# automerge/automerge-classic

Measured on AMD Instinct MI355X. Metric: CRDT ops/sec applied (bulk replay), higher is better.
Workload: dtype u32

## Files before the change

### automerge_classic_amd/csrc/am355_api.hip

```cpp
#include "am355_ctx.h"
#include "am355_scan.h"
#include "am355_textrec.h"

static bool ctx_init(am355_ctx* c) {
  {
    unsigned hw = std::thread::hardware_concurrency();
    const char* env = getenv("AM355_HOST_THREADS");
    unsigned want = env && atoi(env) > 0 ? (unsigned)atoi(env) : std::min(hw ? hw : 4u, 64u);
    c->pool.reset(new HostPool(want > 1 ? want - 1 : 0));
  }
  int prio_low = 0, prio_high = 0;
  (void)hipDeviceGetStreamPriorityRange(&prio_low, &prio_high);
  auto make_stream = [](Stream& s, int prio) { return hipStreamCreateWithPriority(&s.h, hipStreamNonBlocking, prio) == hipSuccess; };
  if (!make_stream(c->stream, prio_high)) return false;
  {
    const char* env = getenv("AM355_HASH_CUS");
    int want = env ? atoi(env) : 0;
    bool made = false;
    if (want > 0) {
      hipDeviceProp_t prop;
      if (hipGetDeviceProperties(&prop, c->device) == hipSuccess && prop.multiProcessorCount > want) {
        int n_cu = prop.multiProcessorCount;
        std::vector<uint32_t> mask((size_t)(n_cu + 31) / 32, 0u);
        for (int k = 0; k < want; k++) { int cu = n_cu - 1 - k; mask[(size_t)cu / 32] |= 1u << (cu % 32); }
        made = hipExtStreamCreateWithCUMask(&c->stream2.h, (uint32_t)mask.size(), mask.data()) == hipSuccess;
      }
    }
    if (!made && !make_stream(c->stream2, prio_low)) return false;
  }
  if (!make_stream(c->stream3, prio_high) || !make_stream(c->stream4, prio_high)) return false;
  for (Event* e : {&c->ev_fork, &c->ev_join, &c->ev[0], &c->ev[1], &c->ev[2], &c->ev[3], &c->ev[4], &c->ev[5], &c->ev[6], &c->ev[7], &c->ev_parse, &c->ev_b0, &c->ev_b1,
                   &c->ev_counts, &c->ev_runs, &c->ev_s1, &c->ev_plan, &c->ev_tables, &c->ev_fills, &c->ev_sched})
    if (hipEventCreate(&e->h) != hipSuccess) return false;
  if (!c->h_sig.ensure(sizeof(HostSignals))) return false;
  memset(c->h_sig.p, 0, sizeof(HostSignals));
  if (const char* e = getenv("AM355_PHASE_EVENTS")) c->phase_events = strcmp(e, "0") != 0;
  return true;
}

extern "C" am355_ctx* am355_create(int device) {
  int n = 0;
  if (hipGetDeviceCount(&n) != hipSuccess || n <= 0 || device < 0 || device >= n) return nullptr;
  (void)hipSetDeviceFlags(hipDeviceScheduleSpin);
  if (hipSetDevice(device) != hipSuccess) return nullptr;
  am355_ctx* c = new am355_ctx();
  c->device = device;
  if (!ctx_init(c)) { delete c; return nullptr; }
  return c;
}

am355_ctx::~am355_ctx() {
  (void)hipSetDevice(device);
  if (lane) lane->wait();
  (void)doc_sum.wait();
  for (const Stream* s : {&stream, &stream2, &stream3, &stream4})
    if (s->h) (void)hipStreamSynchronize(s->h);
  if (shard_comm) (void)am355_shard_finalize(this);
}

extern "C" void am355_destroy(am355_ctx* c) {
  delete c;
}

extern "C" const char* am355_last_error(const am355_ctx* c) { return c ? c->err.c_str() : "no context (no GPU?)"; }
extern "C" uint32_t am355_flags(const am355_ctx* c) { return c ? c->flags : 0; }

extern "C" int am355_set_phase_events(am355_ctx* c, int on) {
  if (!c) return AM355_E_ARG;
  c->phase_events = on != 0;
  return AM355_OK;
}

extern "C" int am355_get_stats(const am355_ctx* c, am355_stats* out) {
  if (!c || !out) return AM355_E_ARG;
  *out = c->stats;
  return AM355_OK;
}

extern "C" int am355_get_hashes(const am355_ctx* c, uint8_t* out) {
  if (!c || !out) return AM355_E_ARG;
  if (!c->replayed || !c->h_hashes.p || c->is_document) return AM355_E_STATE;
  memcpy(out, c->h_hashes.p, 32 * (size_t)c->n_changes);
  return AM355_OK;
}

extern "C" int am355_arena_epoch(const am355_ctx* c, uint64_t* epoch) {
  if (!c || !epoch) return AM355_E_ARG;
  *epoch = c->arena_epoch;
  return AM355_OK;
}

extern "C" int am355_get_hashes_range(const am355_ctx* c, uint32_t first, uint32_t count, uint8_t* out) {
  if (!c || (!out && count)) return AM355_E_ARG;
  if (!c->replayed || !c->h_hashes.p || c->is_document) return AM355_E_STATE;
  if (first > c->n_changes || count > c->n_changes - first) return AM355_E_ARG;
  if (count) memcpy(out, (const uint8_t*)c->h_hashes.p + 32 * (size_t)first, 32 * (size_t)count);
  return AM355_OK;
}

extern "C" int am355_applied_in_input_order(const am355_ctx* c, int* yes) {
  if (!c || !yes) return AM355_E_ARG;
  if (!c->replayed || c->is_document) return AM355_E_STATE;
  bool ok = c->pending_change.empty() && c->n_pending == 0 && c->applied_change.size() == c->n_changes;
  for (uint32_t i = 0; ok && i < c->n_changes; i++) ok = c->applied_change[i] == i;
  *yes = ok ? 1 : 0;
  return AM355_OK;
}

extern "C" int am355_resident_counters(const am355_ctx* c, uint64_t out[3]) {
  if (!c || !out) return AM355_E_ARG;
  out[0] = c->n_resident_calls;
  out[1] = c->n_resident_fallbacks;
  out[2] = c->n_resorder_calls;
  return AM355_OK;
}
// ... 477 lines not shown
```

### automerge_classic_amd/csrc/am355_ctx.h

```cpp
#pragma once
#include "../../include/am355.h"
#include "am355_decode.h"
#include "am355_merge.h"
#include "am355_bigcol.h"
#include "am355_encode.h"
#include "am355_prims.h"
#include "am355_render.h"
#include "am355_host.h"
#include "am355_pinflate.h"
#include "am355_history.h"
#include "am355_delta.h"
#include "am355_resorder.h"
#include "am355_apply.h"
#include "am355_sync.h"
#include "am355_sched.h"
#include "am355_hist.h"
#include "am355_canary.h"

#include <zlib.h>

#include <algorithm>
#include <atomic>
#include <chrono>
#include <cstdarg>
// ... 255 lines not shown
  TraceLap(const char* prefix_, int width_, std::chrono::steady_clock::time_point t0_ = std::chrono::steady_clock::now())
      : on(getenv("AM355_TRACE") != nullptr), prefix(prefix_), width(width_), t0(t0_) {}
  void operator()(const char* what) const {
    if (on) fprintf(stderr, "%s %-*s +%8.3f ms\n", prefix, width, what, std::chrono::duration<double, std::milli>(std::chrono::steady_clock::now() - t0).count());
  }
};

struct SignalBlock {
  static constexpr uint32_t WORDS = 8;
  HostBuf h;
  uint32_t seq = 0;
  bool ready() { return h.ensure((WORDS + 1) * 4); }
  const uint32_t* words() { return h.as<uint32_t>(); }
  hipError_t fetch(const uint32_t* dev, uint32_t n, uint32_t k, hipStream_t st) {
    uint32_t* hw = h.as<uint32_t>();
    volatile uint32_t* hseq = hw + WORDS;
    if (seq == 0) *hseq = 0;
    launch_signal_words(dev, n, nullptr, 0, hw + k, hseq, ++seq, st);
    return wait_host_signal(hseq, seq, st) ? hipSuccess : hipMemcpy(hw + k, dev, 4 * (size_t)n, hipMemcpyDeviceToHost);
  }
};

struct LaneJoin {
  AsyncLane* l = nullptr;
  ~LaneJoin() { if (l) l->wait(); }
};

struct Hash32 {
  uint8_t b[32];
  bool operator==(const Hash32& o) const { return memcmp(b, o.b, 32) == 0; }
};
struct Hash32Hasher {
  size_t operator()(const Hash32& h) const { size_t v; memcpy(&v, h.b, sizeof v); return v; }
};

}
using namespace am355_host;

struct am355_ctx {
  ~am355_ctx();
  int device = 0;
  Stream stream;
  Stream stream2;
  Stream stream3;
  Stream stream4;
  Event ev_fork, ev_join;
  Event ev[8];
  Event ev_parse, ev_b0, ev_b1;
  Event ev_counts, ev_runs;
  std::string err;
  uint32_t flags = 0;

  PinnedBytes raw;
  std::unique_ptr<HostPool> pool;
  std::unique_ptr<AsyncLane> lane;
  std::vector<uint64_t> raw_off;
  uint32_t n_changes = 0;
  DevBuf d_plan_totals;
  bool spec_launched = false;
  bool spec_large_launched = false;
  uint32_t spec_cap_ops = 0, spec_cap_preds = 0;
  uint32_t hint_ops = 0, hint_preds = 0, hint_large = 0;
  bool staged = false, replayed = false, ir_fetched = false;
  int ir_copy_enqueued = 0;
  bool prefetch_ir = false;
  bool has_unknown_cols = false;
  bool staging_in_flight = false;
  bool is_document = false;
  ChangeMeta doc_meta{};
  std::vector<uint32_t> doc_actor_rank;
  DevBuf d_arena, d_offsets, d_metas;
  uint64_t arena_epoch = 1;
  CopyRanges pending_up;
  std::vector<uint32_t> breaks_dev;
  void* breaks_dev_ptr = nullptr;
  HostBuf h_breaks_ahead;
  bool offsets_on_device = false;
  HostBuf h_metas, h_offsets, h_sig;
  uint32_t sig_seq = 0;
  Event ev_s1;
  Event ev_fills;
  Event ev_sched;
  Event ev_plan, ev_tables;
  void* counts_zeroed_at = nullptr; size_t counts_zeroed = 0;
  bool phase_events = false;
  DevBuf d_big, d_bigvals, d_ks;
  HostBuf h_biginfo;
  BigColDesc doc_cols{};
  bool doc_serial = false;
  DevBuf d_entries, d_amap_base, d_amap_prov, d_slots, d_first_idx, d_hashes, d_hash_tab, d_min_idx, d_has_dep, d_words, d_slot_rank, d_scan1, d_plan_sums, d_dep_idx, d_self_idx, d_rank_ids;
  HostBuf h_dep_idx, h_self_idx, h_amap, h_amap_base;
  HostBuf h_slots, h_hashes, h_has_dep, h_words, h_stage, h_s1;
  DevBuf d_s1;
  ChangeBrief* hp_briefs = nullptr;
  uint32_t* hp_distinct = nullptr;
  bool have_host_metas = false;
  uint32_t amap_cap = 0, slot_mask = 0, hash_mask = 0;
  bool used_fast_path = false;

  std::vector<ChangePlan> plans;
  std::vector<uint32_t> applied_change, applied_op_base;
  struct DocSum {
    static constexpr size_t PIECE = (size_t)4 << 20;
    std::thread t;
    std::unique_ptr<std::atomic<uint8_t>[]> copied;
    size_t n_pieces = 0;
    bool pending = false, ok = false;
    bool wait() {
      if (t.joinable()) t.join();
      pending = false;
      return ok;
    }
    ~DocSum() { if (t.joinable()) t.join(); }
  } doc_sum;
  std::vector<uint8_t> doc_bytes;
  std::vector<uint8_t> saved;
  HistoryOutput history;
  bool history_ok = false; uint32_t history_flags = 0;
  std::vector<std::vector<uint8_t>> inflate_scratch;
  std::vector<std::unique_ptr<PInflateJob>> pinflate_jobs;
  std::vector<uint32_t> doc_col_rows;
  std::vector<std::pair<uint32_t, std::vector<uint8_t>>> doc_chg_cols;
  std::vector<uint8_t> doc_tail;
  bool doc_other_ops_cols = false;
  DevBuf d_save, d_enc, d_encout;
  HostBuf h_encout;
  std::vector<uint32_t> amap;
  std::vector<ActorSpan> spans;
  std::vector<uint32_t> actor_tab_off;
  std::vector<std::string> actors;
  std::vector<uint32_t> clock_actor;
  std::vector<uint64_t> clock_seq;
  std::vector<uint8_t> heads;
  uint32_t n_applied = 0, n_pending = 0;
  uint64_t n_ops = 0, n_preds = 0, max_op = 0;
  DevBuf d_plans, d_amap, d_tables;
  ActorSpan* p_spans = nullptr;
  uint32_t* p_tab_off = nullptr;

  DevBuf d_cols, d_pred, d_merge, d_sort, d_ir, d_counts;
  OpCols cols{};
  MergeBufs mb{};
  PatchIR ir{};
  HostBuf h_counts;
  Counts counts{};

  HostBuf h_ir, h_rows;
  am355_patch_ir hir{};
  std::vector<uint32_t> actor_off;
  std::vector<uint8_t> actor_bytes;
  std::string json;

  am355_stats stats{};

  std::vector<uint32_t> pending_change;
  std::vector<uint32_t> pass_first_row;
  DevBuf d_delta, d_pass, d_delta_edit, d_sched, d_hist;
  HostBuf h_sched;
  bool key_unbounded = false;
  bool device_scheduled = false;
  HostBuf h_delta;
  DeltaBufs delta{};
  bool h_tables_current = false, h_tables_were_current = false;
  bool batch_list_only = false;
  void* apply_tail = nullptr;
  ApplyPatch apply;
// ... 207 lines not shown
```

### automerge_classic_amd/csrc/am355_stage.hip

```cpp
#include "am355_ctx.h"
#include "am355_pinflate.h"

bool read_uleb_host(const uint8_t* p, size_t len, size_t& off, uint64_t& out) {
  uint64_t v = 0;
  int shift = 0;
  while (off < len && shift < 64) {
    uint8_t b = p[off++];
    v |= (uint64_t)(b & 0x7f) << shift;
    shift += 7;
    if (!(b & 0x80)) { out = v; return true; }
  }
  return false;
}

constexpr size_t INFLATE_CAP = 0xfff00000ull;

int flush_uploads(am355_ctx* c) {
  if (!c->pending_up.n) return AM355_OK;
  launch_copy_ranges(c->pending_up, c->stream);
  c->pending_up.n = 0;
  HIPCHK(c, hipGetLastError());
  return AM355_OK;
}

int queue_upload(am355_ctx* c, void* dst, const void* src, size_t bytes) {
  if (!bytes) return AM355_OK;
  static const bool off = getenv("AM355_NO_UPLOAD_QUEUE") != nullptr;
  if (off || bytes > ((size_t)256 << 10)) {
    int rc = flush_uploads(c);
    if (rc) return rc;
    HIPCHK(c, hipMemcpyAsync(dst, src, bytes, hipMemcpyHostToDevice, c->stream));
    return AM355_OK;
  }
  if (c->pending_up.n == LAUNCH_RANGES) { int rc = flush_uploads(c); if (rc) return rc; }
  if (!c->pending_up.add(dst, src, bytes)) return fail(c, AM355_E_DEVICE, "upload queue full");
  return AM355_OK;
}

int upload_offsets(am355_ctx* c) {
  if (c->offsets_on_device) return AM355_OK;
  const size_t bytes = sizeof(uint64_t) * ((size_t)c->n_changes + 1);
  if (!c->d_offsets.ensure(bytes) || !c->h_offsets.ensure(bytes)) return fail(c, AM355_E_NOMEM, "device allocation failed");
  memcpy(c->h_offsets.p, c->raw_off.data(), bytes);
  HIPCHK(c, hipMemcpyAsync(c->d_offsets.p, c->h_offsets.p, bytes, hipMemcpyHostToDevice, c->stream));
  c->offsets_on_device = true;
  return AM355_OK;
}

int load_changes_impl(am355_ctx* c, const uint8_t* arena, const uint64_t* offsets, uint32_t n, bool keep_staged) {
  if (!c || (!arena && n) || !offsets) return c ? fail(c, AM355_E_ARG, "null argument") : AM355_E_ARG;
  (void)hipSetDevice(c->device);
  (void)c->doc_sum.wait();
  const uint32_t k0 = keep_staged ? c->n_changes : 0;
  const size_t b0 = keep_staged ? c->raw.size() : 0;
  { int frc = flush_uploads(c); if (frc) return frc; }
  if (c->staging_in_flight) { c->staging_in_flight = false; HIPCHK(c, hipStreamSynchronize(c->stream)); }
  c->staged = c->replayed = c->ir_fetched = false;
  if (!keep_staged) { c->resident_valid = false; c->arena_epoch++; }
  c->apply_ready = false;
  c->state_checked = false;
  c->is_document = false;
  c->flags = 0;
  if (n && offsets[n] - offsets[0] >= ((uint64_t)1 << 20))
    c->pool->prewake(offsets[1] - offsets[0] > 9 && arena[offsets[0] + 8] == 2 ? c->pool->size() : 4);
  for (uint32_t i = 0; i < n; i++)
    if (offsets[i] > offsets[i + 1]) return fail(c, AM355_E_ARG, "change offsets must be ascending (offsets[%u] > offsets[%u])", i, i + 1);
  if (offsets[n] - offsets[0] + b0 >= INFLATE_CAP) { c->flags |= AM355_F_OVERFLOW; return fail(c, AM355_E_UNSUPPORTED, "batch larger than 4 GiB (32-bit arena offsets)"); }
  const size_t in_bytes = (size_t)(offsets[n] - offsets[0]);
  const bool trace = getenv("AM355_TRACE") != nullptr;
  auto t_begin = std::chrono::steady_clock::now();
  auto lap = [&](const char* what) {
    if (trace) fprintf(stderr, "load_changes: %-22s +%8.3f ms\n", what, std::chrono::duration<double, std::milli>(std::chrono::steady_clock::now() - t_begin).count());
  };
  unsigned n_slices = 1;
  const char* slice_env = getenv("AM355_SLICE_BYTES");
  const size_t slice_bytes = slice_env && atol(slice_env) > 0 ? (size_t)atol(slice_env) : (size_t)1 << 21;
  const bool deflated = n && ((offsets[1] - offsets[0] > 9 && arena[offsets[0] + 8] == 2) || (offsets[n / 2 + 1] - offsets[n / 2] > 9 && arena[offsets[n / 2] + 8] == 2));
  const size_t per_slice = deflated && !slice_env ? (size_t)64 << 10 : slice_bytes;
  if (in_bytes >= 2 * per_slice && n >= 16)
    n_slices = (unsigned)std::min<size_t>({(size_t)(c->pool->size() + 1) * (deflated ? 8 : 2), in_bytes / per_slice, (size_t)n / 8});
  if (n_slices < 1) n_slices = 1;
  struct Slice { uint32_t c0 = 0, c1 = 0; size_t out_bytes = 0, base = 0; bool any_deflated = false; int err = 0; uint32_t err_change = 0; std::vector<uint8_t> tmp; std::vector<uint32_t> tmp_len; };
  std::vector<Slice> slices(n_slices);
  {
    uint32_t ci = 0;
    for (unsigned k = 0; k < n_slices; k++) {
      slices[k].c0 = ci;
      uint64_t target = offsets[0] + (uint64_t)in_bytes * (k + 1) / n_slices;
      while (ci < n && (k + 1 == n_slices || offsets[ci + 1] <= target)) ci++;
      slices[k].c1 = ci;
    }
    slices[n_slices - 1].c1 = n;
  }
  auto phase_a = [&](unsigned k) {
    Slice& sl = slices[k];
    for (uint32_t i = sl.c0; i < sl.c1; i++) {
      size_t len = (size_t)(offsets[i + 1] - offsets[i]);
      if (len > 9 && arena[offsets[i] + 8] == 2) { sl.any_deflated = true; break; }
    }
    if (!sl.any_deflated) { sl.out_bytes = (size_t)(offsets[sl.c1] - offsets[sl.c0]); return; }
    sl.tmp_len.resize(sl.c1 - sl.c0);
    std::vector<uint8_t> out;
    for (uint32_t i = sl.c0; i < sl.c1 && !sl.err; i++) {
      const uint8_t* p = arena + offsets[i];
      size_t len = (size_t)(offsets[i + 1] - offsets[i]);
      size_t before = sl.tmp.size();
      if (len > 9 && p[8] == 2) {
        size_t off = 9;
        uint64_t clen;
        if (!read_uleb_host(p, len, off, clen) || clen > len - off) { sl.err = 10; sl.err_change = i; break; }
        int irc = inflate_raw(p + off, (size_t)clen, out, INFLATE_CAP);
        if (irc) { sl.err = irc; sl.err_change = i; break; }
        sl.tmp.insert(sl.tmp.end(), p, p + 8);
        sl.tmp.push_back(1);
        uint64_t v = out.size();
        do { uint8_t x = v & 0x7f; v >>= 7; if (v) x |= 0x80; sl.tmp.push_back(x); } while (v);
        sl.tmp.insert(sl.tmp.end(), out.begin(), out.end());
      } else {
        sl.tmp.insert(sl.tmp.end(), p, p + len);
      }
      if (sl.tmp.size() >= INFLATE_CAP) { sl.err = 2; sl.err_change = i; break; }
      sl.tmp_len[i - sl.c0] = (uint32_t)(sl.tmp.size() - before);
    }
    sl.out_bytes = sl.tmp.size();
  };
  c->pool->run(n_slices, phase_a);
  lap("inflate / sizes");
  size_t total = 0;
  for (Slice& sl : slices) {
    if (sl.err == 10) { c->flags |= AM355_F_BAD_CHUNK; return fail(c, AM355_E_INVALID, "change %u: bad deflate container", sl.err_change); }
    if (sl.err == 3) return fail(c, AM355_E_NOMEM, "inflate: out of memory");
    if (sl.err == 2) { c->flags |= AM355_F_OVERFLOW; return fail(c, AM355_E_UNSUPPORTED, "change %u: inflated size beyond the 4 GiB batch limit", sl.err_change); }
    if (sl.err) { c->flags |= AM355_F_BAD_DEFLATE; return fail(c, AM355_E_INVALID, "change %u: invalid or truncated deflate data", sl.err_change); }
    sl.base = total;
    total += sl.out_bytes;
    if (total + b0 >= INFLATE_CAP) { c->flags |= AM355_F_OVERFLOW; return fail(c, AM355_E_UNSUPPORTED, "batch larger than 4 GiB (32-bit arena offsets)"); }
  }
  const uint32_t n_all = k0 + n;
  c->raw.resize(b0 + total);
  c->raw_off.resize((size_t)n_all + 1);
  c->raw_off[n_all] = b0 + total;
  c->n_changes = n_all;
  if (!(keep_staged ? c->d_arena.ensure_keep(b0 + total + 64, b0) : c->d_arena.ensure(total + 64)) || !c->d_offsets.ensure(sizeof(uint64_t) * ((size_t)n_all + 1)) ||
      !(keep_staged ? c->d_metas.ensure_keep(sizeof(ChangeMeta) * (size_t)std::max(n_all, 1u), sizeof(ChangeMeta) * (size_t)k0)
                    : c->d_metas.ensure(sizeof(ChangeMeta) * (size_t)std::max(n_all, 1u))) || !c->h_metas.ensure(sizeof(ChangeMeta) * (size_t)std::max(n_all, 1u)) ||
      !c->d_counts.ensure(sizeof(Counts)) || !c->h_counts.ensure(2 * sizeof(Counts)) || !c->h_offsets.ensure(sizeof(uint64_t) * ((size_t)n_all + 1)))
    return fail(c, AM355_E_NOMEM, "device allocation failed");
  uint8_t* raw = c->raw.data() + b0;
  uint8_t* d_raw = c->d_arena.as<uint8_t>() + b0;
  uint64_t* roff = c->raw_off.data() + k0;
  std::vector<hipError_t> h2d(n_slices, hipSuccess);
  bool any_deflated = false;
  for (const Slice& sl : slices) any_deflated = any_deflated || sl.any_deflated;
  const char* gather_env = getenv("AM355_GATHER_UNIT");
  if (!any_deflated && (total >= ((size_t)4 << 20) || (gather_env && total > 0))) {
    const size_t unit = gather_env && atol(gather_env) > 0 ? (size_t)atol(gather_env) : (size_t)256 << 10;
    const size_t n_units = (total + unit - 1) / unit;
    std::vector<uint32_t> group_of(n_units);
    std::vector<size_t> group_first;
    for (size_t u = 0, span = 1; u < n_units; span = std::min<size_t>(span * 2, 64)) {
      group_first.push_back(u);
      for (size_t k = 0; k < span && u < n_units; k++, u++) group_of[u] = (uint32_t)group_first.size() - 1;
    }
    const size_t n_groups = group_first.size();
    group_first.push_back(n_units);
    std::vector<std::atomic<uint32_t>> left(n_groups);
    for (size_t g = 0; g < n_groups; g++) left[g].store((uint32_t)(group_first[g + 1] - group_first[g]));
    h2d.assign(n_groups, hipSuccess);
    const uint8_t* src = arena + offsets[0];
    const uint64_t off0 = offsets[0];
    std::atomic<size_t> next_unit{0};
    const unsigned n_helpers = (unsigned)std::min<size_t>(4, std::min<size_t>(n_units > 1 ? n_units - 1 : 0, c->pool->size()));
    lap("  buffers ready");
    c->pool->run(n_helpers + 1, [&](unsigned task) {
      const bool issuer = task == 0;
      size_t next_group = 0;
      auto issue_ready = [&]() {
        while (next_group < n_groups && left[next_group].load(std::memory_order_acquire) == 0) {
          size_t gb = group_first[next_group] * unit, ge = std::min(total, group_first[next_group + 1] * unit);
          h2d[next_group] = hipMemcpyAsync(d_raw + gb, raw + gb, ge - gb, hipMemcpyHostToDevice, c->stream);
          if (trace) fprintf(stderr, "load_changes:   group %zu (%zu KiB) enqueued +%8.3f ms\n", next_group, (ge - gb) >> 10, std::chrono::duration<double, std::milli>(std::chrono::steady_clock::now() - t_begin).count());
          next_group++;
        }
      };
      if (issuer) (void)hipSetDevice(c->device);
      for (;;) {
        size_t u = next_unit.fetch_add(1, std::memory_order_relaxed);
        if (u >= n_units) break;
        size_t b = u * unit, e = std::min(total, b + unit);
        memcpy(raw + b, src + b, e - b);
        left[group_of[u]].fetch_sub(1, std::memory_order_acq_rel);
        if (issuer) issue_ready();
      }
      if (issuer) {
        while (next_group < n_groups) {
          issue_ready();
#if defined(__x86_64__)
          __builtin_ia32_pause();
#endif
        }
      }
    });
    for (uint32_t i = 0; i < n; i++) roff[i] = b0 + (offsets[i] - off0);
  } else {
    std::vector<uint32_t> group_of(n_slices);
    std::vector<size_t> group_begin{0};
    {
      size_t acc = 0;
      for (unsigned k = 0; k < n_slices; k++) {
        group_of[k] = (uint32_t)group_begin.size() - 1;
        acc += slices[k].out_bytes;
        if (acc >= ((size_t)2 << 20) && k + 1 < n_slices) { group_begin.push_back(slices[k + 1].base); acc = 0; }
      }
      group_begin.push_back(total);
    }
    const size_t n_groups = group_begin.size() - 1;
    std::vector<std::atomic<uint32_t>> left(n_groups);
    for (auto& x : left) x.store(0);
    for (unsigned k = 0; k < n_slices; k++) left[group_of[k]].fetch_add(1);
    h2d.assign(n_groups, hipSuccess);
    if (n_slices == 1) {
      Slice& sl = slices[0];
      if (sl.any_deflated) {
        if (sl.out_bytes) memcpy(raw, sl.tmp.data(), sl.out_bytes);
        size_t o = b0;
        for (uint32_t i = 0; i < n; i++) { roff[i] = o; o += sl.tmp_len[i]; }
      } else {
        if (sl.out_bytes) memcpy(raw, arena + offsets[0], sl.out_bytes);
        for (uint32_t i = 0; i < n; i++) roff[i] = b0 + (offsets[i] - offsets[0]);
      }
      if (total) {
        if (keep_staged) { int qrc = queue_upload(c, d_raw, raw, total); if (qrc) return qrc; }
        else h2d[0] = hipMemcpyAsync(d_raw, raw, total, hipMemcpyHostToDevice, c->stream);
      }
    } else
    c->pool->run(n_slices + 1, [&](unsigned task) {
      if (task == 0) {
        (void)hipSetDevice(c->device);
        for (size_t g = 0; g < n_groups; g++) {
          while (left[g].load(std::memory_order_acquire) != 0) {
#if defined(__x86_64__)
            __builtin_ia32_pause();
#endif
          }
          size_t gb = group_begin[g], ge = group_begin[g + 1];
          if (ge > gb) h2d[g] = hipMemcpyAsync(d_raw + gb, raw + gb, ge - gb, hipMemcpyHostToDevice, c->stream);
        }
        return;
      }
      Slice& sl = slices[task - 1];
      if (sl.any_deflated) {
        if (sl.out_bytes) memcpy(raw + sl.base, sl.tmp.data(), sl.out_bytes);
        size_t o = b0 + sl.base;
        for (uint32_t i = sl.c0; i < sl.c1; i++) { roff[i] = o; o += sl.tmp_len[i - sl.c0]; }
      } else {
        if (sl.out_bytes) memcpy(raw + sl.base, arena + offsets[sl.c0], sl.out_bytes);
        for (uint32_t i = sl.c0; i < sl.c1; i++) roff[i] = b0 + sl.base + (offsets[i] - offsets[sl.c0]);
      }
      left[group_of[task - 1]].fetch_sub(1, std::memory_order_acq_rel);
    });
  }
  lap("gathered, H2D enqueued");
  for (hipError_t e : h2d)
    if (e != hipSuccess) return fail(c, AM355_E_DEVICE, "hipMemcpyAsync (arena): %s", hipGetErrorString(e));
  c->offsets_on_device = false;
  if (!keep_staged) { int orc = upload_offsets(c); if (orc) return orc; }
  c->staging_in_flight = true;
  static const bool stage_sync = getenv("AM355_STAGE_SYNC") != nullptr;
  if (trace || stage_sync) { c->staging_in_flight = false; HIPCHK(c, hipStreamSynchronize(c->stream)); lap("H2D done"); }
  c->staged = true;
  c->stats = am355_stats{};
  c->stats.n_changes = n_all;
  c->stats.raw_bytes = c->raw.size();
  return AM355_OK;
}

namespace {
struct HostRle {
  const uint8_t* p; size_t len, off = 0; int64_t count = 0; int state = 0; int64_t last = 0; bool last_null = true; bool is_signed;
  HostRle(const uint8_t* p_, size_t l, bool sg) : p(p_), len(l), is_signed(sg) {}
  bool done() const { return count == 0 && off >= len; }
  bool leb(bool sg, int64_t& out) {
    uint64_t v = 0; int shift = 0;
    while (off < len && shift < 64) {
      uint8_t b = p[off++];
// ... 391 lines not shown
```

### automerge_classic_amd/engine.py

```python
import ctypes
import os

import numpy as np

_HERE = os.path.dirname(os.path.abspath(__file__))
DEFAULT_LIB = os.path.join(_HERE, "csrc", "libam355.so")

AM355_OK = 0
AM355_E_DEVICE, AM355_E_ARG, AM355_E_INVALID, AM355_E_UNSUPPORTED, AM355_E_STATE, AM355_E_NOMEM = -1, -2, -3, -4, -5, -6

FLAG_NAMES = {
    1 << 0: "BAD_MAGIC", 1 << 1: "BAD_CHECKSUM", 1 << 2: "BAD_CHUNK", 1 << 3: "BAD_COLUMNS", 1 << 4: "BAD_LEB", 1 << 5: "BAD_RLE",
    1 << 6: "BAD_ROW", 1 << 7: "UNKNOWN_OBJECT", 1 << 8: "BAD_ELEM", 1 << 9: "BAD_PRED", 1 << 10: "DUP_OPID", 1 << 11: "BAD_COUNTER",
    1 << 12: "UNSUPPORTED", 1 << 13: "OVERFLOW", 1 << 16: "BAD_SEQ", 1 << 17: "UNKNOWN_ACTOR", 1 << 18: "BAD_DEFLATE",
}


class Stats(ctypes.Structure):
    _fields_ = [
        ("n_changes", ctypes.c_uint32), ("n_applied", ctypes.c_uint32), ("n_pending", ctypes.c_uint32),
        ("n_actors", ctypes.c_uint32), ("n_objects", ctypes.c_uint32), ("n_heads", ctypes.c_uint32),
        ("n_ops", ctypes.c_uint64), ("max_op", ctypes.c_uint64), ("raw_bytes", ctypes.c_uint64),
        ("n_map_values", ctypes.c_uint64), ("n_list_elems", ctypes.c_uint64), ("n_edits", ctypes.c_uint64),
        ("ir_bytes", ctypes.c_uint64),
# ... 327 lines not shown
        L.am355_resident_new_actor_calls.restype = ctypes.c_int
    if hasattr(L, "am355_set_resident_new_objects"):
        L.am355_set_resident_new_objects.argtypes = [vp, ctypes.c_int]
        L.am355_set_resident_new_objects.restype = ctypes.c_int
        L.am355_resident_new_object_calls.argtypes = [vp, vp]
        L.am355_resident_new_object_calls.restype = ctypes.c_int
    if hasattr(L, "am355_set_resident_counters"):
        L.am355_set_resident_counters.argtypes = [vp, ctypes.c_int]
        L.am355_set_resident_counters.restype = ctypes.c_int
        L.am355_resident_counter_calls.argtypes = [vp, vp]
        L.am355_resident_counter_calls.restype = ctypes.c_int
    if hasattr(L, "am355_set_resident_map_merge"):
        L.am355_set_resident_map_merge.argtypes = [vp, ctypes.c_int]
        L.am355_set_resident_map_merge.restype = ctypes.c_int
        L.am355_resident_map_merge_calls.argtypes = [vp, vp]
        L.am355_resident_map_merge_calls.restype = ctypes.c_int
    if hasattr(L, "am355_apply_local_change"):
        L.am355_encode_change.argtypes = [vp, ctypes.POINTER(LocalChange), ctypes.POINTER(ctypes.c_void_p), ctypes.POINTER(ctypes.c_size_t), vp]
        L.am355_apply_local_change.argtypes = [vp, ctypes.POINTER(LocalChange), ctypes.POINTER(ctypes.c_void_p), ctypes.POINTER(ctypes.c_size_t)]
        L.am355_local_change_calls.argtypes = [vp, vp]
        for f in ("am355_encode_change", "am355_apply_local_change", "am355_local_change_calls"):
            getattr(L, f).restype = ctypes.c_int
    if hasattr(L, "am355_set_local_small"):
        L.am355_set_local_small.argtypes = [vp, ctypes.c_int]
        L.am355_set_local_small.restype = ctypes.c_int
        L.am355_local_small_calls.argtypes = [vp, vp]
        L.am355_local_small_calls.restype = ctypes.c_int
    if hasattr(L, "am355_changes_added"):
        L.am355_find_changes.argtypes = [vp, vp, u32, vp]
        for f in ("am355_changes_since", "am355_changes_added", "am355_missing_deps"):
            getattr(L, f).argtypes = [vp, vp, u32, ctypes.POINTER(ctypes.c_void_p), ctypes.POINTER(u32)]
        L.am355_set_graph_probe_min.argtypes = [vp, u32]
        L.am355_graph_query_calls.argtypes = [vp, vp]
        L.am355_test_hash_probe.argtypes = [vp, vp, u32, vp, u32, vp]
        for f in ("am355_find_changes", "am355_changes_since", "am355_changes_added", "am355_missing_deps", "am355_set_graph_probe_min", "am355_graph_query_calls",
                  "am355_test_hash_probe"):
            getattr(L, f).restype = ctypes.c_int
    if hasattr(L, "am355_object_text"):
        L.am355_object_text.argtypes = [vp, ctypes.c_uint64, vp, ctypes.c_size_t, ctypes.POINTER(ctypes.c_void_p), ctypes.POINTER(ctypes.c_size_t), ctypes.POINTER(TextInfo)]
        L.am355_object_text_calls.argtypes = [vp, vp]
        L.am355_set_text_pinned_max.argtypes = [vp, ctypes.c_uint64]
        L.am355_text_limits.argtypes = [vp]
        for f in ("am355_object_text", "am355_object_text_calls", "am355_set_text_pinned_max", "am355_text_limits"):
            getattr(L, f).restype = ctypes.c_int
    if hasattr(L, "am355_text_splice"):
        L.am355_text_locate.argtypes = [vp, ctypes.c_uint64, vp, ctypes.c_size_t, ctypes.c_uint64, ctypes.c_uint64, ctypes.POINTER(ctypes.c_void_p), ctypes.POINTER(u32),
                                        ctypes.POINTER(ctypes.c_uint64)]
        L.am355_text_splice.argtypes = [vp, ctypes.c_uint64, vp, ctypes.c_size_t, ctypes.c_uint64, ctypes.c_uint64, vp, vp, u32, vp, ctypes.c_size_t, ctypes.c_int64, vp, u32,
                                        ctypes.POINTER(ctypes.c_void_p), ctypes.POINTER(ctypes.c_size_t)]
        L.am355_text_splice_calls.argtypes = [vp, vp]
        L.am355_text_locate_limits.argtypes = [vp]
        for f in ("am355_text_locate", "am355_text_splice", "am355_text_splice_calls", "am355_text_locate_limits"):
            getattr(L, f).restype = ctypes.c_int
    if hasattr(L, "am355_list_splice"):
        pvp, psz = ctypes.POINTER(ctypes.c_void_p), ctypes.POINTER(ctypes.c_size_t)
        L.am355_list_locate.argtypes = [vp, ctypes.c_uint64, vp, ctypes.c_size_t, ctypes.c_uint64, ctypes.c_uint64, pvp, ctypes.POINTER(u32), pvp, ctypes.POINTER(u32),
                                        ctypes.POINTER(ctypes.c_uint64)]
        L.am355_list_splice.argtypes = [vp, ctypes.c_uint64, vp, ctypes.c_size_t, ctypes.c_uint64, ctypes.c_uint64, vp, u32, vp, u32, vp, ctypes.c_size_t, ctypes.c_int64, vp, u32,
                                        pvp, psz]
        L.am355_list_set.argtypes = [vp, ctypes.c_uint64, vp, ctypes.c_size_t, ctypes.c_uint64, vp, vp, u32, vp, ctypes.c_size_t, ctypes.c_int64, vp, u32, pvp, psz]
        L.am355_list_splice_calls.argtypes = [vp, vp]
        L.am355_list_locate_limits.argtypes = [vp]
        L.am355_test_list_premises.argtypes = [vp, vp, u32, u32, u32, u32, ctypes.POINTER(u32), ctypes.POINTER(u32)]
        for f in ("am355_list_locate", "am355_list_splice", "am355_list_set", "am355_list_splice_calls", "am355_list_locate_limits", "am355_test_list_premises"):
            getattr(L, f).restype = ctypes.c_int
    if hasattr(L, "am355_text_position"):
        L.am355_text_position.argtypes = [vp, ctypes.c_uint64, vp, ctypes.c_size_t, vp, u32, ctypes.POINTER(ctypes.c_void_p), ctypes.POINTER(ctypes.c_uint64)]
        L.am355_rank_of_actor.argtypes = [vp, vp, ctypes.c_size_t, ctypes.POINTER(u32)]
        L.am355_actor_of_rank.argtypes = [vp, u32, ctypes.POINTER(ctypes.c_void_p), ctypes.POINTER(ctypes.c_size_t)]
        L.am355_actor_of_rank.restype = ctypes.c_int
        L.am355_text_position_calls.argtypes = [vp, vp]
        L.am355_text_position_limits.argtypes = [vp]
        for f in ("am355_text_position", "am355_rank_of_actor", "am355_text_position_calls", "am355_text_position_limits"):
            getattr(L, f).restype = ctypes.c_int
    if hasattr(L, "am355_map_update"):
        pvp, psz = ctypes.POINTER(ctypes.c_void_p), ctypes.POINTER(ctypes.c_size_t)
        L.am355_map_locate.argtypes = [vp, ctypes.c_uint64, vp, ctypes.c_size_t, vp, vp, u32, pvp, pvp, ctypes.POINTER(u32)]
        L.am355_map_update.argtypes = [vp, ctypes.c_uint64, vp, ctypes.c_size_t, vp, u32, vp, u32, vp, u32, vp, ctypes.c_size_t, ctypes.c_int64, vp, u32, pvp, psz]
        L.am355_map_calls.argtypes = [vp, vp]
        L.am355_map_locate_limits.argtypes = [vp]
        L.am355_set_map_locate_thread.argtypes = [vp, ctypes.c_int]
        for f in ("am355_map_locate", "am355_map_update", "am355_map_calls", "am355_map_locate_limits", "am355_set_map_locate_thread"):
            getattr(L, f).restype = ctypes.c_int
    L.am355_get_raw.argtypes = [vp, ctypes.POINTER(ctypes.c_void_p), ctypes.POINTER(ctypes.c_void_p), ctypes.POINTER(u32)]
    L.am355_doc_changes.argtypes = [vp, u32, ctypes.POINTER(ctypes.c_void_p), ctypes.POINTER(ctypes.c_void_p), ctypes.POINTER(u32), ctypes.POINTER(ctypes.c_void_p)]
    L.am355_apply_changes.argtypes = [vp, vp, u64p, u32]
    L.am355_apply_patch_json.argtypes = [vp, ctypes.POINTER(ctypes.c_char_p), ctypes.POINTER(ctypes.c_size_t)]
    L.am355_fetch_apply_ir.argtypes = [vp, vp]
    L.am355_reset.argtypes = [vp]
    L.am355_get_dep_graph.argtypes = [vp, ctypes.POINTER(ctypes.c_void_p), ctypes.POINTER(ctypes.c_void_p), ctypes.POINTER(u32)]
    L.am355_sync_bloom_build.argtypes = [vp, vp, u32, vp, ctypes.c_size_t]
    L.am355_sync_bloom_probe.argtypes = [vp, vp, u32, u32, u32, u32, vp, ctypes.c_size_t, vp]
    L.am355_get_pending.argtypes = [vp, vp, ctypes.POINTER(u32)]
    L.am355_forget_call_history.argtypes = [vp, ctypes.c_int]
    L.am355_hash_graph_known.argtypes = [vp, ctypes.c_int, ctypes.POINTER(ctypes.c_int)]
    L.am355_set_phase_events.argtypes = [vp, ctypes.c_int]
    for f in ("am355_load_changes", "am355_load_document", "am355_replay", "am355_patch_json", "am355_get_stats", "am355_get_hashes", "am355_test_sort",
              "am355_test_scan", "am355_get_rows", "am355_save", "am355_get_applied", "am355_fetch_ir", "am355_get_raw", "am355_set_shard", "am355_fragment_size", "am355_export_fragment",
              "am355_import_fragments", "am355_doc_changes", "am355_apply_changes", "am355_apply_patch_json", "am355_fetch_apply_ir", "am355_reset", "am355_get_pending", "am355_forget_call_history", "am355_hash_graph_known", "am355_set_phase_events", "am355_get_dep_graph", "am355_sync_bloom_build", "am355_sync_bloom_probe"):
        getattr(L, f).restype = ctypes.c_int
    return L


_libs = {}


def load_library(path=DEFAULT_LIB):
    if path not in _libs:
        _libs[path] = _bind(path)
    return _libs[path]


class Engine:

    def __init__(self, device=0, lib_path=DEFAULT_LIB):
        self._L = load_library(lib_path)
        self.device = device
        self.lib_path = lib_path
        self._h = self._L.am355_create(device)
        if not self._h:
            raise RuntimeError("am355_create failed: no usable MI355X / HIP device (the engine has no CPU fallback)")
        self._n_changes = 0

    def set_phase_events(self, on):
        self._check(self._L.am355_set_phase_events(self._h, 1 if on else 0))

    def close(self):
        if getattr(self, "_h", None):
            self._L.am355_destroy(self._h)
            self._h = None

    def __del__(self):
        try:
            self.close()
        except Exception:
            pass

    def _check(self, rc):
        if rc == AM355_OK:
            return
        msg = self._L.am355_last_error(self._h).decode("utf-8", "replace")
        flags = self._L.am355_flags(self._h)
        cls = InvalidChanges if rc == AM355_E_INVALID else UnsupportedChanges if rc == AM355_E_UNSUPPORTED else EngineError
        raise cls(rc, msg, flags)

    def load_changes(self, log):
        arena = np.ascontiguousarray(log.arena, dtype=np.uint8)
        offsets = np.ascontiguousarray(log.offsets, dtype=np.uint64)
        self._n_changes = int(offsets.size - 1)
        self._check(self._L.am355_load_changes(self._h, arena.ctypes.data if arena.size else None, offsets.ctypes.data, self._n_changes))

    def load_document(self, doc: bytes):
        buf = np.frombuffer(bytes(doc), dtype=np.uint8)
        self._n_changes = 0
        self._check(self._L.am355_load_document(self._h, buf.ctypes.data, buf.size))

    def backend_load(self, doc: bytes):
        buf = doc if isinstance(doc, np.ndarray) else np.frombuffer(bytes(doc), dtype=np.uint8)
        self._n_changes = 0
        self._check(self._L.am355_backend_load(self._h, buf.ctypes.data, buf.size))

    def replay(self):
        self._check(self._L.am355_replay(self._h))

    def apply_changes(self, log):
        arena = np.ascontiguousarray(log.arena, dtype=np.uint8)
        offsets = np.ascontiguousarray(log.offsets, dtype=np.uint64)
        self._check(self._L.am355_apply_changes(self._h, arena.ctypes.data if arena.size else None, offsets.ctypes.data, int(offsets.size - 1)))
        self._n_changes = int(self.stats().n_changes)

    def encode_change(self, request):
        lc, keep = flatten_change_request(request)
        p, n, h = ctypes.c_void_p(), ctypes.c_size_t(), (ctypes.c_uint8 * 32)()
        self._check(self._L.am355_encode_change(self._h, ctypes.byref(lc), ctypes.byref(p), ctypes.byref(n), h))
        del keep
        return ctypes.string_at(p, n.value), bytes(h)

    def apply_local_change(self, request):
        lc, keep = flatten_change_request(request)
        p, n = ctypes.c_void_p(), ctypes.c_size_t()
        self._check(self._L.am355_apply_local_change(self._h, ctypes.byref(lc), ctypes.byref(p), ctypes.byref(n)))
        del keep
        self._n_changes = int(self.stats().n_changes)
        return ctypes.string_at(p, n.value)

    def local_change_calls(self):
        out = (ctypes.c_uint64 * 2)()
        self._check(self._L.am355_local_change_calls(self._h, out))
        return int(out[0]), int(out[1])

    def set_local_small(self, on):
        self._check(self._L.am355_set_local_small(self._h, 1 if on else 0))

# ... 618 lines not shown
```

### include/am355.h

```cpp
#ifndef AM355_H
#define AM355_H
#include <stddef.h>
#include <stdint.h>

#ifdef __cplusplus
extern "C" {
#endif

typedef struct am355_ctx am355_ctx;

enum {
  AM355_OK = 0,
  AM355_E_DEVICE = -1,
  AM355_E_ARG = -2,
  AM355_E_INVALID = -3,
  AM355_E_UNSUPPORTED = -4,
  AM355_E_STATE = -5,
  AM355_E_NOMEM = -6
};

enum {
  AM355_F_BAD_MAGIC = 1u << 0, AM355_F_BAD_CHECKSUM = 1u << 1, AM355_F_BAD_CHUNK = 1u << 2, AM355_F_BAD_COLUMNS = 1u << 3,
  AM355_F_BAD_LEB = 1u << 4, AM355_F_BAD_RLE = 1u << 5, AM355_F_BAD_ROW = 1u << 6, AM355_F_UNKNOWN_OBJECT = 1u << 7,
  AM355_F_BAD_ELEM = 1u << 8, AM355_F_BAD_PRED = 1u << 9, AM355_F_DUP_OPID = 1u << 10, AM355_F_BAD_COUNTER = 1u << 11,
// ... 199 lines not shown
int am355_object_text_calls(const am355_ctx *ctx, uint64_t out[2]);
int am355_set_text_pinned_max(am355_ctx *ctx, uint64_t bytes);
int am355_text_limits(uint32_t out[4]);

enum { AM355_RUN_COUNTER = 1u };
typedef struct { uint32_t elem_ctr, elem_actor, pred_ctr, pred_actor, count, flags; } am355_text_run;
int am355_text_locate(am355_ctx *ctx, uint64_t obj_ctr, const uint8_t *obj_actor, size_t actor_len,
                      uint64_t first, uint64_t n, const am355_text_run **runs, uint32_t *n_runs, uint64_t *length);
int am355_text_splice(am355_ctx *ctx, uint64_t obj_ctr, const uint8_t *obj_actor, size_t actor_len,
                      uint64_t start, uint64_t deletions,
                      const uint8_t *utf8, const uint32_t *value_off, uint32_t n_values,
                      const uint8_t *author, size_t author_len, int64_t time, const uint8_t *message, uint32_t message_len,
                      const uint8_t **change, size_t *len);
int am355_text_splice_calls(const am355_ctx *ctx, uint64_t out[3]);
int am355_text_locate_limits(uint32_t out[3]);
int am355_actor_of_rank(const am355_ctx *ctx, uint32_t rank, const uint8_t **bytes, size_t *len);

typedef struct { uint32_t elem_ctr, elem_actor, count, flags, pred_first, pred_num; } am355_list_run;
typedef struct { uint32_t actor, ctr; } am355_list_pred;
int am355_list_locate(am355_ctx *ctx, uint64_t obj_ctr, const uint8_t *obj_actor, size_t actor_len, uint64_t first, uint64_t n,
                      const am355_list_run **runs, uint32_t *n_runs, const am355_list_pred **preds, uint32_t *n_preds, uint64_t *length);
int am355_list_splice(am355_ctx *ctx, uint64_t obj_ctr, const uint8_t *obj_actor, size_t actor_len, uint64_t start, uint64_t deletions,
                      const am355_local_value *values, uint32_t n_values, const uint8_t *strings, uint32_t strings_len,
                      const uint8_t *author, size_t author_len, int64_t time, const uint8_t *message, uint32_t message_len,
                      const uint8_t **change, size_t *len);
int am355_list_set(am355_ctx *ctx, uint64_t obj_ctr, const uint8_t *obj_actor, size_t actor_len, uint64_t index,
                   const am355_local_value *value, const uint8_t *strings, uint32_t strings_len,
                   const uint8_t *author, size_t author_len, int64_t time, const uint8_t *message, uint32_t message_len,
                   const uint8_t **change, size_t *len);
int am355_list_splice_calls(const am355_ctx *ctx, uint64_t out[3]);
int am355_list_locate_limits(uint32_t out[3]);

enum { AM355_MOP_SET = 1, AM355_MOP_DELETE = 2, AM355_MOP_INC = 3 };
typedef struct { uint32_t first, num, flags, pad; } am355_map_hit;
typedef struct {
  uint32_t kind;
  uint32_t key_off, key_len;
  uint32_t value;
  int64_t delta;
} am355_map_op;
int am355_map_locate(am355_ctx *ctx, uint64_t obj_ctr, const uint8_t *obj_actor, size_t actor_len,
                     const uint8_t *keys, const uint32_t *key_off, uint32_t n,
                     const am355_map_hit **hits, const am355_ir_map **recs, uint32_t *n_recs);
int am355_map_update(am355_ctx *ctx, uint64_t obj_ctr, const uint8_t *obj_actor, size_t actor_len,
                     const am355_map_op *ops, uint32_t n_ops, const uint8_t *strings, uint32_t strings_len,
                     const am355_local_value *values, uint32_t n_values,
                     const uint8_t *author, size_t author_len, int64_t time, const uint8_t *message, uint32_t message_len,
                     const uint8_t **change, size_t *len);
int am355_map_calls(const am355_ctx *ctx, uint64_t out[3]);
int am355_map_locate_limits(uint32_t out[4]);
int am355_set_map_locate_thread(am355_ctx *ctx, int on);

enum { AM355_POS_UNKNOWN = 0u, AM355_POS_VISIBLE = 1u, AM355_POS_DELETED = 2u, AM355_POS_STATUS = 3u , AM355_POS_COUNTER = 0x100u };
typedef struct { uint32_t ctr, actor; } am355_elem_id;
typedef struct { uint32_t position, status; } am355_elem_pos;
int am355_text_position(am355_ctx *ctx, uint64_t obj_ctr, const uint8_t *obj_actor, size_t actor_len,
                        const am355_elem_id *ids, uint32_t n, const am355_elem_pos **out, uint64_t *length);
int am355_rank_of_actor(const am355_ctx *ctx, const uint8_t *bytes, size_t len, uint32_t *rank);
int am355_text_position_calls(const am355_ctx *ctx, uint64_t out[2]);
int am355_text_position_limits(uint32_t out[2]);

int am355_test_hash_probe(am355_ctx *ctx, const uint8_t *table_hashes, uint32_t n_table, const uint8_t *queries, uint32_t n_queries, uint32_t *out_idx);
int am355_test_sort(am355_ctx *ctx, uint64_t *keys, uint32_t *vals, uint32_t n, int key_bits);
int am355_test_scan(am355_ctx *ctx, const uint32_t *in, uint32_t *out, uint32_t n, uint32_t *total);
int am355_test_scan_at(am355_ctx *ctx, uint32_t *in_buf, uint32_t in_words, uint32_t in_off, uint32_t *out_buf, uint32_t out_words, uint32_t out_off,
                       uint32_t n, uint32_t *total);
int am355_test_scan2(am355_ctx *ctx, uint32_t *in_a, uint32_t *in_b, uint32_t in_words, uint32_t in_off, uint32_t *out_a, uint32_t *out_b, uint32_t out_words,
                     uint32_t out_off, uint32_t n, uint32_t *total_a, uint32_t *total_b);
int am355_test_scan_terminators(am355_ctx *ctx, const uint8_t *bytes_buf, size_t bytes_len, uint32_t byte_off, uint32_t L, uint32_t *out_buf, uint32_t out_words,
                                uint32_t out_off, uint32_t *total);
int am355_test_max(am355_ctx *ctx, const uint32_t *v, uint32_t n, uint32_t *inout);
int am355_test_sort_bits(am355_ctx *ctx, uint64_t *keys, uint32_t *vals, uint32_t n, int begin_bit, int end_bit, const uint32_t *first_table, int *result_buffer);
int am355_test_chain_mark(am355_ctx *ctx, const uint32_t *next, uint32_t *mark, uint32_t mark_words, uint32_t n);
int am355_test_remap(am355_ctx *ctx, uint32_t *buf, uint32_t words, uint32_t base_off, const uint32_t *ranges, uint32_t n_ranges, const uint32_t *table, uint32_t n_old,
                     uint32_t *n_added);
int am355_test_fill(am355_ctx *ctx, uint32_t *buf, uint32_t words, uint32_t base_off, const uint32_t *ranges, uint32_t n_ranges, uint32_t *n_added);
int am355_test_copy(am355_ctx *ctx, uint8_t *dst, size_t dst_bytes, const uint8_t *src, size_t src_bytes, int src_pinned, const uint32_t *ranges, uint32_t n_ranges,
                    uint32_t *n_added);
int am355_test_signal_words(am355_ctx *ctx, const uint32_t *a, uint32_t n_a, const uint32_t *b, uint32_t n_b, uint32_t seq, uint32_t *host_words, uint32_t host_words_n,
                            uint32_t *seq_word);
int am355_test_carried_scan(am355_ctx *ctx, const uint32_t *v, uint32_t n, uint32_t *out, uint32_t *out_wg, uint32_t *wg_total);
int am355_test_text_premises(am355_ctx *ctx, const am355_ir_edit *table, uint32_t n_recs, uint32_t begin, uint32_t R, uint32_t n_values, uint32_t *flags, uint32_t *length);
int am355_test_list_premises(am355_ctx *ctx, const am355_ir_edit *table, uint32_t n_recs, uint32_t begin, uint32_t R, uint32_t n_values, uint32_t *flags, uint32_t *length);
int am355_get_rows(am355_ctx *ctx, uint32_t *obj_actor, uint32_t *obj_ctr, uint32_t *key_actor, uint32_t *key_ctr, uint32_t *key_off,
                   uint32_t *key_len, uint32_t *action, uint32_t *val_tl, uint32_t *val_off, uint32_t *pred_num, uint32_t *id_ctr,
                   uint32_t *id_actor, uint8_t *insert, uint32_t *succ_cnt);

#ifdef __cplusplus
}
#endif
#endif
```

Baseline: 1.257 billion.

## Split staged host-to-device uploads across two streams and halve the tail group

The staged arena upload groups now alternate between the main stream and a second high-priority stream, so consecutive group copies can be in flight at the same time. The main stream then waits on an event recorded on the second stream. The grouping is also changed so the last groups split the remaining units in half instead of making one large final group, which shortens the copy left after the host gather finishes. The cost is extra cross-stream synchronisation, and the gain may be limited if a single copy already saturates the PCIe link.

```diff
diff --git a/automerge_classic_amd/csrc/am355_api.hip b/automerge_classic_amd/csrc/am355_api.hip
--- a/automerge_classic_amd/csrc/am355_api.hip
+++ b/automerge_classic_amd/csrc/am355_api.hip
@@ -30,7 +30,7 @@
   }
   if (!make_stream(c->stream3, prio_high) || !make_stream(c->stream4, prio_high)) return false;
   for (Event* e : {&c->ev_fork, &c->ev_join, &c->ev[0], &c->ev[1], &c->ev[2], &c->ev[3], &c->ev[4], &c->ev[5], &c->ev[6], &c->ev[7], &c->ev_parse, &c->ev_b0, &c->ev_b1,
-                   &c->ev_counts, &c->ev_runs, &c->ev_s1, &c->ev_plan, &c->ev_tables, &c->ev_fills, &c->ev_sched})
+                   &c->ev_counts, &c->ev_runs, &c->ev_s1, &c->ev_plan, &c->ev_tables, &c->ev_fills, &c->ev_sched, &c->ev_stage})
     if (hipEventCreate(&e->h) != hipSuccess) return false;
   if (!c->h_sig.ensure(sizeof(HostSignals))) return false;
   memset(c->h_sig.p, 0, sizeof(HostSignals));
diff --git a/automerge_classic_amd/csrc/am355_ctx.h b/automerge_classic_amd/csrc/am355_ctx.h
--- a/automerge_classic_amd/csrc/am355_ctx.h
+++ b/automerge_classic_amd/csrc/am355_ctx.h
@@ -361,6 +361,7 @@
   Event ev_fills;
   Event ev_sched;
   Event ev_plan, ev_tables;
+  Event ev_stage;
   void* counts_zeroed_at = nullptr; size_t counts_zeroed = 0;
   bool phase_events = false;
   DevBuf d_big, d_bigvals, d_ks;
diff --git a/automerge_classic_amd/csrc/am355_stage.hip b/automerge_classic_amd/csrc/am355_stage.hip
--- a/automerge_classic_amd/csrc/am355_stage.hip
+++ b/automerge_classic_amd/csrc/am355_stage.hip
@@ -44,6 +44,30 @@
   memcpy(c->h_offsets.p, c->raw_off.data(), bytes);
   HIPCHK(c, hipMemcpyAsync(c->d_offsets.p, c->h_offsets.p, bytes, hipMemcpyHostToDevice, c->stream));
   c->offsets_on_device = true;
+  return AM355_OK;
+}
+
+constexpr size_t STAGE_UNIT = (size_t)256 << 10, STAGE_CAP_UNITS = 64, STAGE_TAIL_UNITS = STAGE_CAP_UNITS / 2;
+static std::vector<size_t> stage_groups(size_t total, size_t unit) {
+  const size_t n_units = (total + unit - 1) / unit, cap = STAGE_CAP_UNITS, tail = STAGE_TAIL_UNITS;
+  std::vector<size_t> first;
+  for (size_t u = 0, span = 1; u < n_units; span = std::min(span * 2, cap)) {
+    const size_t left = n_units - u;
+    first.push_back(u);
+    u += left > span ? span : left > tail ? left - left / 2 : left;
+  }
+  first.push_back(n_units);
+  return first;
+}
+
+extern "C" int am355_test_stage_groups(uint64_t total, uint64_t unit, uint64_t* first_unit, uint32_t cap, uint32_t* n_groups, uint32_t limits[3]) {
+  if (!n_groups || !limits) return AM355_E_ARG;
+  limits[0] = (uint32_t)STAGE_UNIT; limits[1] = (uint32_t)STAGE_CAP_UNITS; limits[2] = (uint32_t)STAGE_TAIL_UNITS;
+  if (!unit) unit = STAGE_UNIT;
+  const std::vector<size_t> first = stage_groups((size_t)total, (size_t)unit);
+  *n_groups = (uint32_t)first.size() - 1;
+  if (first.size() > cap) return first_unit ? AM355_E_ARG : AM355_OK;
+  for (size_t g = 0; g < first.size(); g++) first_unit[g] = first[g];
   return AM355_OK;
 }
 
@@ -154,16 +178,13 @@
   for (const Slice& sl : slices) any_deflated = any_deflated || sl.any_deflated;
   const char* gather_env = getenv("AM355_GATHER_UNIT");
   if (!any_deflated && (total >= ((size_t)4 << 20) || (gather_env && total > 0))) {
-    const size_t unit = gather_env && atol(gather_env) > 0 ? (size_t)atol(gather_env) : (size_t)256 << 10;
-    const size_t n_units = (total + unit - 1) / unit;
+    const size_t unit = gather_env && atol(gather_env) > 0 ? (size_t)atol(gather_env) : STAGE_UNIT;
+    const bool one_lane = getenv("AM355_STAGE_ONE_LANE") != nullptr;
+    const std::vector<size_t> group_first = stage_groups(total, unit);
+    const size_t n_units = group_first.back(), n_groups = group_first.size() - 1;
     std::vector<uint32_t> group_of(n_units);
-    std::vector<size_t> group_first;
-    for (size_t u = 0, span = 1; u < n_units; span = std::min<size_t>(span * 2, 64)) {
-      group_first.push_back(u);
-      for (size_t k = 0; k < span && u < n_units; k++, u++) group_of[u] = (uint32_t)group_first.size() - 1;
-    }
-    const size_t n_groups = group_first.size();
-    group_first.push_back(n_units);
+    for (size_t g = 0; g < n_groups; g++)
+      for (size_t u = group_first[g]; u < group_first[g + 1]; u++) group_of[u] = (uint32_t)g;
     std::vector<std::atomic<uint32_t>> left(n_groups);
     for (size_t g = 0; g < n_groups; g++) left[g].store((uint32_t)(group_first[g + 1] - group_first[g]));
     h2d.assign(n_groups, hipSuccess);
@@ -178,7 +199,7 @@
       auto issue_ready = [&]() {
         while (next_group < n_groups && left[next_group].load(std::memory_order_acquire) == 0) {
           size_t gb = group_first[next_group] * unit, ge = std::min(total, group_first[next_group + 1] * unit);
-          h2d[next_group] = hipMemcpyAsync(d_raw + gb, raw + gb, ge - gb, hipMemcpyHostToDevice, c->stream);
+          h2d[next_group] = hipMemcpyAsync(d_raw + gb, raw + gb, ge - gb, hipMemcpyHostToDevice, (next_group & 1) || one_lane ? c->stream : c->stream4);
           if (trace) fprintf(stderr, "load_changes:   group %zu (%zu KiB) enqueued +%8.3f ms\n", next_group, (ge - gb) >> 10, std::chrono::duration<double, std::milli>(std::chrono::steady_clock::now() - t_begin).count());
           next_group++;
         }
@@ -201,6 +222,11 @@
         }
       }
     });
+    if (!one_lane) {
+      hipError_t e = hipEventRecord(c->ev_stage, c->stream4);
+      if (e == hipSuccess) e = hipStreamWaitEvent(c->stream, c->ev_stage, 0);
+      if (e != hipSuccess) h2d.push_back(e);
+    }
     for (uint32_t i = 0; i < n; i++) roff[i] = b0 + (offsets[i] - off0);
   } else {
     std::vector<uint32_t> group_of(n_slices);
diff --git a/automerge_classic_amd/engine.py b/automerge_classic_amd/engine.py
--- a/automerge_classic_amd/engine.py
+++ b/automerge_classic_amd/engine.py
@@ -433,6 +433,9 @@
         L.am355_set_map_locate_thread.argtypes = [vp, ctypes.c_int]
         for f in ("am355_map_locate", "am355_map_update", "am355_map_calls", "am355_map_locate_limits", "am355_set_map_locate_thread"):
             getattr(L, f).restype = ctypes.c_int
+    if hasattr(L, "am355_test_stage_groups"):
+        L.am355_test_stage_groups.argtypes = [ctypes.c_uint64, ctypes.c_uint64, vp, u32, ctypes.POINTER(u32), ctypes.POINTER(u32)]
+        L.am355_test_stage_groups.restype = ctypes.c_int
     L.am355_get_raw.argtypes = [vp, ctypes.POINTER(ctypes.c_void_p), ctypes.POINTER(ctypes.c_void_p), ctypes.POINTER(u32)]
     L.am355_doc_changes.argtypes = [vp, u32, ctypes.POINTER(ctypes.c_void_p), ctypes.POINTER(ctypes.c_void_p), ctypes.POINTER(u32), ctypes.POINTER(ctypes.c_void_p)]
     L.am355_apply_changes.argtypes = [vp, vp, u64p, u32]
@@ -460,6 +463,19 @@
     if path not in _libs:
         _libs[path] = _bind(path)
     return _libs[path]
+
+
+def stage_groups(total, unit=0, lib_path=DEFAULT_LIB):
+    L = load_library(lib_path)
+    n, limits = ctypes.c_uint32(0), (ctypes.c_uint32 * 3)()
+    rc = L.am355_test_stage_groups(total, unit, None, 0, ctypes.byref(n), limits)
+    if rc != AM355_OK:
+        raise EngineError(rc, "am355_test_stage_groups", 0)
+    first = np.zeros(n.value + 1, dtype=np.uint64)
+    rc = L.am355_test_stage_groups(total, unit, first.ctypes.data, first.size, ctypes.byref(n), limits)
+    if rc != AM355_OK:
+        raise EngineError(rc, "am355_test_stage_groups", 0)
+    return [int(x) for x in first], {"unit": limits[0], "cap_units": limits[1], "tail_units": limits[2]}
 
 
 class Engine:
diff --git a/include/am355.h b/include/am355.h
--- a/include/am355.h
+++ b/include/am355.h
@@ -305,6 +305,7 @@
 int am355_test_carried_scan(am355_ctx *ctx, const uint32_t *v, uint32_t n, uint32_t *out, uint32_t *out_wg, uint32_t *wg_total);
 int am355_test_text_premises(am355_ctx *ctx, const am355_ir_edit *table, uint32_t n_recs, uint32_t begin, uint32_t R, uint32_t n_values, uint32_t *flags, uint32_t *length);
 int am355_test_list_premises(am355_ctx *ctx, const am355_ir_edit *table, uint32_t n_recs, uint32_t begin, uint32_t R, uint32_t n_values, uint32_t *flags, uint32_t *length);
+int am355_test_stage_groups(uint64_t total, uint64_t unit, uint64_t *first_unit, uint32_t cap, uint32_t *n_groups, uint32_t limits[3]);
 int am355_get_rows(am355_ctx *ctx, uint32_t *obj_actor, uint32_t *obj_ctr, uint32_t *key_actor, uint32_t *key_ctr, uint32_t *key_off,
                    uint32_t *key_len, uint32_t *action, uint32_t *val_tl, uint32_t *val_off, uint32_t *pred_num, uint32_t *id_ctr,
                    uint32_t *id_actor, uint8_t *insert, uint32_t *succ_cnt);
```

Result: slower. 1.144 billion (-9.0%).
